# IIT-PAVIS/Acoustic-Image-Generation

Hardware: AMD Instinct MI355X
Metric: train-step images/sec (higher is better)
Workload: dtype f32

## Files before the change

acoustic-image-generation_amd/acimg/_lib.py:

```python
import ctypes as C
import os

_HERE = os.path.dirname(os.path.abspath(__file__))
LIB_PATH = os.environ.get("ACIMG_LIB") or os.path.join(_HERE, "lib", "libacimg.so")

ACT_NONE, ACT_RELU, ACT_SIGMOID = 0, 1, 2


class ConvDesc(C.Structure):

    _fields_ = [(n, C.c_int32) for n in (
        "N", "H", "W", "C", "ldx", "K", "ldy", "OH", "OW", "R", "S", "stride", "pad_t", "pad_l",
        "ldw", "act")]

    def __repr__(self):
        return "ConvDesc(" + ", ".join("%s=%d" % (n, getattr(self, n)) for n, _ in self._fields_) + ")"


class Config(C.Structure):

    _fields_ = [(n, C.c_int32) for n in (
        "splitk_cut", "splitk_target", "splitk_handoff", "wgrad_minpix", "wgrad_halo", "split3_tile_bm",
        "split3_tile_bn", "tail_split", "tail_s", "trunk_persistent", "trunk_bk", "trunk_stagger", "trunk_dma_pos",
        "trunk_ring", "trunk_ring_bm", "trunk_halo")]
# ... 29 lines not shown
    "acimg_conv2d_fwd_tiling": (_I, [_DP, C.POINTER(C.c_int)]),
    "acimg_config_default": (_I, [C.POINTER(Config)]),
    "acimg_configure": (_I, [C.POINTER(Config)]),
    "acimg_conv2d_fwd_workspace": (_SZ, [_DP]),
    "acimg_conv2d_split3_weight_bytes": (_SZ, [_DP]),
    "acimg_conv2d_split3_prepare": (_I, [_DP, _P, _P, _P]),
    "acimg_conv2d_bf16_prepare": (_I, [_DP, _P, _P, _P]),
    "acimg_conv2d_fwd_split3_stats_rows": (_I, [_DP]),
    "acimg_conv2d_fwd_split3_tiling": (_I, [_DP, C.POINTER(C.c_int)]),
    "acimg_conv2d_fwd_split3p_stats_rows": (_I, [_DP]),
    "acimg_conv2d_fwd_split3": (_I, [_DP, _P, _P, _P, _P, _P, _P, _I, _P, _P]),
    "acimg_conv2d_fwd_bf16": (_I, [_DP, _P, _P, _P, _P, _P, _P, _I, _P, _P]),
    "acimg_conv2d_split3_dgrad_weight_bytes": (_SZ, [_DP]),
    "acimg_conv2d_split3_prepare_dgrad": (_I, [_DP, _P, _P, _P]),
    "acimg_conv2d_dgrad_split3": (_I, [_DP, _P, _I, _P, _P, _I, _P, _I, _P, _I, _P]),
    "acimg_conv2d_dgrad_bf16": (_I, [_DP, _P, _I, _P, _P, _I, _P, _I, _P, _I, _P]),
    "acimg_conv2d_split3_prepare_multi": (_I, [_I, _P, _P, _P, _P, _P]),
    "acimg_conv2d_fwd_split3p_workspace": (_SZ, [_DP]),
    "acimg_conv2d_fwd_split3p": (_I, [_DP, _P, _SZ, _P, _P, _P, _P, _SZ, _P]),
    "acimg_conv2d_fwd_split1p": (_I, [_DP, _P, _SZ, _P, _P, _P, _P, _SZ, _P]),
    "acimg_conv2d_fwd_split3p_stats": (_I, [_DP, _P, _SZ, _P, _P, _P, _SZ, _P]),
    "acimg_gram_stats_workspace": (_SZ, [_L, _I]),
    "acimg_gram_stats": (_I, [_P, _SZ, _L, _I, _P, _I, _I, _P, _P, _P, _P, _F, _F, _P, _P, _P, _SZ, _P]),
    "acimg_conv2d_fwd_split3p_tail": (_I, [_DP, _P, _SZ, _P, _P, _P, _P, _SZ, _P, _SZ, _P, _SZ, _P]),
    "acimg_conv2d_fwd_split3p_tail_proj": (_I, [_DP, _P, _SZ, _P, _P, _P, _P, _P, _P, _P, _SZ, _P, _SZ, _P]),
    "acimg_split_plane_bytes": (_SZ, [_L, _I]),
    "acimg_bn_relu_split": (_I, [_P, _P, _P, _I, _P, _SZ, _L, _I, _P]),
    "acimg_bn_add_relu_split": (_I, [_P, _P, _P, _P, _P, _P, _P, _SZ, _P, _SZ, _P, _I, _I, _I, _I, _I, _I, _I, _P]),
    "acimg_bn_relu_maxpool_split": (_I, [_P, _P, _P, _P, _SZ, _I, _I, _I, _I, _I, _I, _I, _I, _P]),
    "acimg_conv2d_dgrad": (_I, [_DP, _P, _I, _P, _P, _I, _P, _I, _P, _I, _P, _SZ, _P, _P]),
    "acimg_conv2d_dgrad_workspace": (_SZ, [_DP]),
    "acimg_conv2d_wgrad": (_I, [_DP, _P, _P, _I, _P, _P, _P, _SZ, _P]),
    "acimg_conv2d_wgrad_workspace": (_SZ, [_DP]),
    "acimg_conv2d_wgrad_split3": (_I, [_DP, _P, _P, _I, _P, _P, _P, _SZ, _P]),
    "acimg_conv2d_wgrad_bf16": (_I, [_DP, _P, _P, _I, _P, _P, _P, _SZ, _P]),
    "acimg_conv2d_affine_input_ok": (_I, [_DP, _I]),
    "acimg_conv2d_wgrad_affine": (_I, [_DP, _I, _P, _P, _P, _I, _P, _I, _P, _P, _P, _SZ, _P]),
    "acimg_deconv_fwd": (_I, [_DP, _P, _P, _P, _P, _P, _SZ, _P, _P]),
    "acimg_deconv_dgrad": (_I, [_DP, _P, _I, _P, _P, _P, _I, _P, _SZ, _P, _P]),
    "acimg_deconv_wgrad": (_I, [_DP, _P, _P, _I, _P, _P, _P, _SZ, _P]),
    "acimg_deconv_workspace": (_SZ, [_DP]),
    "acimg_bn_finalize": (_I, [_P, _I, _I, _I, _D, _P, _P, _P, _P, _F, _F, _I, _P, _P, _P, _P, _P]),
    "acimg_bn_add_relu": (_I, [_P, _P, _P, _P, _P, _P, _P, _I, _I, _I, _I, _I, _I, _I, _P]),
    "acimg_bn_relu_maxpool": (_I, [_P, _P, _P, _P, _I, _I, _I, _I, _I, _I, _I, _I, _P]),
    "acimg_bn_relu": (_I, [_P, _P, _P, _P, _L, _I, _I, _I, _P]),
    "acimg_bn_relu_bwd": (_I, [_P, _P, _P, _P, _P, _P, _P, _P, _P, _L, _I, _P]),
# ... 155 lines not shown
```

acoustic-image-generation_amd/acimg/ops.py:

```python
import ctypes as C
import math

import torch

from . import _lib
from ._lib import ACT_NONE, ACT_RELU, ACT_SIGMOID, ConvDesc


def up4(v):
    return (int(v) + 3) & ~3


class Ptr(object):

    __slots__ = ("t", "off")

    def __init__(self, t, off=0):
        self.t = t
        self.off = int(off)

    def addr(self):
        return self.t.data_ptr() + 4 * self.off


# ... 432 lines not shown
    nbytes = 0 if tail_ws is None else (tail_ws.numel() * tail_ws.element_size() if hasattr(tail_ws, "numel") else 0)
    fn = _L().acimg_conv2d_fwd_split3p if terms == 3 else _L().acimg_conv2d_fwd_split1p
    plan.add("conv2d_fwd_split3p" if terms == 3 else "conv2d_fwd_split1p", fn, C.byref(d), x_planes, int(x_lo_off),
             wsplit, y, stats, tail_ws, int(nbytes), side=side)


def conv2d_fwd_split3p_stats(plan, d, x_planes, x_lo_off, wsplit, stats, tail_ws=None, side=False):
    nbytes = 0 if tail_ws is None else (tail_ws.numel() * tail_ws.element_size() if hasattr(tail_ws, "numel") else 0)
    plan.add("conv2d_fwd_split3p_stats", _L().acimg_conv2d_fwd_split3p_stats, C.byref(d), x_planes, int(x_lo_off), wsplit,
             stats, tail_ws, int(nbytes), side=side)


def gram_stats_workspace(rows, Cn):
    return int(_L().acimg_gram_stats_workspace(int(rows), int(Cn)))


def gram_stats(plan, x_planes, x_lo_off, rows, Cn, w, ldw, K, gamma, beta, moving_mean, moving_var, scale, shift, ws,
               decay=0.997, eps=1e-5, side=False):
    plan.add("gram_stats", _L().acimg_gram_stats, x_planes, int(x_lo_off), int(rows), int(Cn), w, int(ldw), int(K), gamma,
             beta, moving_mean, moving_var, float(decay), float(eps), scale, shift, ws,
             int(ws.numel() * ws.element_size()), side=side)


def conv2d_fwd_split3p_tail(plan, d, x_planes, x_lo_off, wsplit, scale, shift, sc_planes, sc_lo_off, out_planes,
                            out_lo_off, tail_ws=None, side=False):
    nbytes = 0 if tail_ws is None else (tail_ws.numel() * tail_ws.element_size() if hasattr(tail_ws, "numel") else 0)
    plan.add("conv2d_fwd_split3p_tail", _L().acimg_conv2d_fwd_split3p_tail, C.byref(d), x_planes, int(x_lo_off), wsplit,
             scale, shift, sc_planes, int(sc_lo_off), out_planes, int(out_lo_off), tail_ws, int(nbytes), side=side)


def conv2d_fwd_split3p_tail_proj(plan, d, x_planes, x_lo_off, wsplit, scale, shift, sc32, sc_scale, sc_shift, out_planes,
                                 out_lo_off, tail_ws=None, side=False):
    nbytes = 0 if tail_ws is None else (tail_ws.numel() * tail_ws.element_size() if hasattr(tail_ws, "numel") else 0)
    plan.add("conv2d_fwd_split3p_tail_proj", _L().acimg_conv2d_fwd_split3p_tail_proj, C.byref(d), x_planes, int(x_lo_off),
             wsplit, scale, shift, sc32, sc_scale, sc_shift, out_planes, int(out_lo_off), tail_ws, int(nbytes), side=side)


def bn_relu_split(plan, x, scale, shift, relu, out, lo_off, rows, Cn):
    plan.add("bn_relu_split", _L().acimg_bn_relu_split, x, scale, shift, int(relu), out, int(lo_off), int(rows), Cn)


def bn_add_relu_split(plan, a, sa, ta, b32, sb, tb, b_planes, b_lo_off, out_planes, out_lo_off, out32, N, OH, OW,
                      Cn, BH, BW, bstride):
    plan.add("bn_add_relu_split", _L().acimg_bn_add_relu_split, a, sa, ta, b32, sb, tb, b_planes, int(b_lo_off),
             out_planes, int(out_lo_off), out32, N, OH, OW, Cn, BH, BW, bstride)

# ... 364 lines not shown
```

acoustic-image-generation_amd/acimg/vision.py:

```python
from collections import OrderedDict, namedtuple

import numpy as np
import torch

from . import ops
from .model import Model, flat_ptr, load_state_file
from .params import Var, up4

BLOCKS = (("block1", 64, 3, 1), ("block2", 128, 4, 2), ("block3", 256, 6, 2), ("block4", 512, 3, 1))
WEIGHT_DECAY = 5e-4
BN_DECAY = 0.997
BN_EPS = 1e-5
PLANE_SLACK = 2 * 15 * 2048 * 2 + 512

Stage = namedtuple("Stage", "tag a b p1 p2 r1 r2 r3 sc")


class ResNet50Model(Model):

    def __init__(self, input_shape=None, num_classes=None, precision="f16x3", stages=None, stage_cut=8, side_lane=True,
                 two_pass=True, two_pass_max_cin=256, gram=True):
        self.scope = 'resnet_v1_50'
        assert precision in ("f16x3", "f32", "f16")
        self.precision = precision
        self._split = precision in ("f16x3", "f16")
        self._terms = 1 if precision == "f16" else 3
        if stages is None:
            stages = 2 if precision in ("f16x3", "f16") else 1
        assert stages in (1, 2)
        if precision not in ("f16x3", "f16"):
            stages = 1
        self.stages = stages
        self.STAGE_CUT = int(stage_cut)
        self.side_lane = bool(side_lane) and stages == 1
        self.two_pass = bool(two_pass) and precision == "f16x3"
        self.two_pass_max_cin = int(two_pass_max_cin)
        self.gram = bool(gram) and self.two_pass
        self._ctor = dict(input_shape=list(input_shape), num_classes=num_classes, precision=precision, stages=stages,
                          stage_cut=int(stage_cut), side_lane=bool(side_lane), two_pass=bool(two_pass),
                          two_pass_max_cin=int(two_pass_max_cin), gram=bool(gram))
        self.num_classes = num_classes
        self.height = input_shape[0]
        self.width = input_shape[1]
        self.channels = input_shape[2]
        if num_classes is not None:
            raise NotImplementedError("the logits layer is not on the acoustic-image path (num_classes=None)")
        self.session = None
        self.output = None
        self.network = None
        self.frozen_calls = None
        self.stage_calls = None
        self.stage_read_calls = None

    def clone_kwargs(self):
        return dict(self._ctor)

    def _units(self):
        depth_in = 64
        for name, base, n, stride in BLOCKS:
            for u in range(n):
                s = stride if u == n - 1 else 1
                yield ("%s/%s/unit_%d/bottleneck_v1" % (self.scope, name, u + 1), depth_in, base * 4, base, s)
                depth_in = base * 4
# ... 200 lines not shown
                 save=False):
        d = ops.conv_desc(self.N, hw[0], hw[1], cin, cout, kh, kw, stride, padding, ldx=cin, ldy=up4(cout),
                          ldw=up4(cout))
        rows = ops.conv2d_stats_rows(d)
        stats = self._lane_stats("", rows * 2 * up4(cout))
        isc, ish = (in_aff if in_aff is not None else (None, None))
        ops.conv2d_fwd(plan, d, x, self._var(scope + "/weights"), None, out, isc, ish, 1, stats if training else None)
        sc, sh = self._bn_finalize(plan, scope, cout, stats, rows, self.N * d.OH * d.OW, training, save=save)
        return d.OH, d.OW, sc, sh

    def _conv_bn_planes(self, plan, scope, xplanes, hw, cin, kh, kw, cout, stride, padding, out, training, side=False,
                        tag=""):
        d = ops.conv_desc(self.N, hw[0], hw[1], cin, cout, kh, kw, stride, padding, ldx=cin, ldy=up4(cout),
                          ldw=up4(cout))
        rows = ops.conv2d_fwd_split3p_stats_rows(d) if self._terms == 3 else ops.conv2d_fwd_split3_stats_rows(d)
        lane = ("_side" if side else "") + tag
        stats = self._lane_stats(lane, rows * 2 * up4(cout))
        tail_ws = self._lane_ws("tail", lane, ops.conv2d_fwd_split3p_workspace(d))
        ops.conv2d_fwd_split3p(plan, d, xplanes, self._lo_off(self.N * hw[0] * hw[1], cin), self._split_image(scope, d),
                               out, stats if training else None, tail_ws=tail_ws, terms=self._terms, side=side)
        sc, sh = self._bn_finalize(plan, scope, cout, stats, rows, self.N * d.OH * d.OW, training, side=side)
        return d.OH, d.OW, sc, sh

    def _conv3_two_pass(self, plan, scope, xplanes, hw, cin, cout, sc_planes, out_planes, training, tag="", proj=None):
        d = ops.conv_desc(self.N, hw[0], hw[1], cin, cout, 1, 1, 1, "SAME", ldx=cin, ldy=cout, ldw=cout)
        M = self.N * hw[0] * hw[1]
        rows = -(-M // 128)
        stats = self._lane_stats(tag, rows * 2 * cout)
        wsplit = self._split_image(scope, d)
        tail_ws = self._lane_ws("tail", tag, ops.conv2d_fwd_split3p_workspace(d))
        lo = self._lo_off(M, cin)
        lo_out = self._lo_off(M, cout)
        if training and self.gram and ops.gram_stats_workspace(M, cin) > 0:
            sc, sh = self._affine(scope, cout)
            b = scope + "/BatchNorm/"
            ops.gram_stats(plan, xplanes, lo, M, cin, self._var(scope + "/weights"), cout, cout, self._var(b + "gamma"),
                           self._var(b + "beta"), self._var(b + "moving_mean"), self._var(b + "moving_variance"), sc, sh,
                           self._lane_ws("gram", tag, ops.gram_stats_workspace(M, cin)), BN_DECAY, BN_EPS)
        else:
            if training:
                ops.conv2d_fwd_split3p_stats(plan, d, xplanes, lo, wsplit, stats, tail_ws=tail_ws)
            sc, sh = self._bn_finalize(plan, scope, cout, stats, rows, M, training)
        if proj is not None:
            ops.conv2d_fwd_split3p_tail_proj(plan, d, xplanes, lo, wsplit, sc, sh, proj[0], proj[1], proj[2], out_planes,
                                             lo_out, tail_ws=tail_ws)
        else:
            ops.conv2d_fwd_split3p_tail(plan, d, xplanes, lo, wsplit, sc, sh, sc_planes, lo_out, out_planes, lo_out,
                                        tail_ws=tail_ws)

    def _two_pass_ok(self, hw, cin, cout):
        M = self.N * hw[0] * hw[1]
        if not (self.two_pass and self._terms == 3 and cin <= self.two_pass_max_cin and cout % 128 == 0 and
                M * cout * 4 < 2 ** 31):
            return False
        d = ops.conv_desc(self.N, hw[0], hw[1], cin, cout, 1, 1, 1, "SAME", ldx=cin, ldy=cout, ldw=cout)
        return tuple(ops.conv2d_fwd_split3_tiling(d)[:2]) == (128, 128)

    def _record_forward_split(self, plan, training):
        N = self.N
        H, W = self.height, self.width
        plan.add_hook(self._refresh_split_weights)
# ... 20 lines not shown
            def shortcut_conv(side):
                _, _, ssc, tsc = self._conv_bn_planes(plan, scope + "/shortcut", cur, (h, w), din, 1, 1, d, s, "SAME",
                                                      st.sc, training, side=side, tag=st.tag)
                return st.sc, ssc, tsc

            beside = din != d and self.side_lane
            if beside:
                plan.fork()
                forked = shortcut_conv(True)

            def shortcut():
                if din == d:
                    return None
                if beside:
                    plan.join()
                    return forked
                return shortcut_conv(False)

            oh1, ow1, s1, t1 = self._conv_bn_planes(plan, scope + "/conv1", cur, (h, w), din, 1, 1, db, 1, "SAME",
                                                    st.r1, training, tag=st.tag)
            ops.bn_relu_split(plan, st.r1, s1, t1, 1, st.p1, self._lo_off(N * h * w, db), N * h * w, db)
            oh2, ow2, s2, t2 = self._conv_bn_planes(plan, scope + "/conv2", st.p1, (h, w), db, 3, 3, db, s,
                                                    "SAME" if s == 1 else 1, st.r2, training, tag=st.tag)
            ops.bn_relu_split(plan, st.r2, s2, t2, 1, st.p2, self._lo_off(N * oh2 * ow2, db), N * oh2 * ow2, db)
            if s == 1 and not last and self._two_pass_ok((oh2, ow2), db, d):
                self._conv3_two_pass(plan, scope + "/conv3", st.p2, (oh2, ow2), db, d, cur, nxt_out, training, tag=st.tag,
                                     proj=shortcut())
            else:
                _, _, s3, t3 = self._conv_bn_planes(plan, scope + "/conv3", st.p2, (oh2, ow2), db, 1, 1, d, 1, "SAME",
                                                    st.r3, training, tag=st.tag)
                out_planes = None if last else nxt_out
                out_lo = 0 if last else self._lo_off(N * oh2 * ow2, d)
                out32 = self.xfinal if last else None
                proj = shortcut()
                if proj is not None:
                    ops.bn_add_relu_split(plan, st.r3, s3, t3, proj[0], proj[1], proj[2], None, 0, out_planes, out_lo,
                                          out32, N, oh2, ow2, d, oh2, ow2, 1)
                else:
                    ops.bn_add_relu_split(plan, st.r3, s3, t3, None, None, None, cur, self._lo_off(N * h * w, din),
                                          out_planes, out_lo, out32, N, oh2, ow2, d, h, w, s)
            h, w = oh2, ow2
            if i == first2:
                if training:
                    self.stage_read_calls = len(plan.calls)
                cur, nxt = st.a, st.b
            else:
                cur, nxt = nxt, cur
        fh, fw = self.feat_hw
        if training:
            self.frozen_calls = len(plan.calls)
# ... 100 lines not shown
```

acoustic-image-generation_amd/csrc/gram.hip:

```cpp
#include "split_planes.hpp"

namespace acimg {

struct GramParams {
    const char* X;
    unsigned x_bytes;
    unsigned lo_off;
    int rows;
    int C;
    int nb;
    int S;
    int steps;
    float* part;
    float* sxpart;
};

template <int NCC>
__device__ __forceinline__ h16x8 gram_frag(const char* region, int ct, int h, int lane) {
    const int t = lane & 15, q = t >> 2, p = t & 3, g = lane >> 4;
    const int brick = ((2 * h + (g >> 1)) * NCC + (ct >> 1)) * 1024;
    const int kc = 2 * (ct & 1) + (p >> 1);
    const int row0 = 8 * (g & 1) + q, row1 = row0 + 4;
    const int a0 = brick + row0 * 64 + ((kc ^ swz(row0)) << 4) + 8 * (p & 1);
    const int a1 = brick + row1 * 64 + ((kc ^ swz(row1)) << 4) + 8 * (p & 1);
    return tr16_frag<h16x8>(region + a0, region + a1);
}

template <int BC>
__global__ __launch_bounds__(512, 2) void gram_partial_kernel(const GramParams p) {
    constexpr int NCC = BC / 32;
    constexpr int KPB = 4;
    constexpr int REG = KPB * NCC * 1024;
    constexpr int NSD = BC == 128 ? 4 : 3, NSN = 3;
    constexpr int WGN = 4;
    constexpr int TM = BC / 2 / 16, TN = BC / WGN / 16;
    constexpr int PWD = 2 * KPB * NCC / 8;
    constexpr int PWN = 3 * KPB * NCC / 8;
    static_assert(BC == 128 || BC == 64, "block side");

    extern __shared__ __attribute__((aligned(16))) float smem[];
    char* const lds = reinterpret_cast<char*>(smem);
    const int tid = threadIdx.x, lane = tid & 63, wid = tid >> 6;
    const int wm = wid / WGN, wn = wid % WGN;
    const int li = lane & 15, g = lane >> 4;

    const int nb2 = p.nb * p.nb;
    const int xcd = blockIdx.x & 7, slot = blockIdx.x >> 3;
    const int s = xcd + 8 * (slot / nb2), b = slot % nb2;
    if (s >= p.S) return;
    const int bi = b / p.nb, bj = b % p.nb;
    const bool diag = BC == 64 || bi == bj;
// ... 17 lines not shown
    const int STAGE = diag ? 2 * REG : 3 * REG;
    int islot = 0;
    auto issue = [&](int t) {
        char* st = lds + islot * STAGE;
        islot = islot + 1 == NS ? 0 : islot + 1;
#pragma unroll
        for (int j = 0; j < PWN; ++j) {
            if (j >= PWD && diag) break;
            const int p16 = pb0 + KPB * t + pc_pb[j];
            const unsigned goff = (t < p.steps && 16 * p16 + (lane >> 2) < p.rows) ? pc_goff[j] + (unsigned)p16 * cpb * 1024u
                                                                                    : OOB;
            char* dst = st + pc_dst[j];
            __builtin_amdgcn_raw_ptr_buffer_load_lds(rs, (lds_ptr_t)dst, 16, goff, 0, 0, 0);
        }
    };

    f32x4 acc[TM][TN], accs[TN];
#pragma unroll
    for (int j = 0; j < TN; ++j) {
        accs[j] = f32x4{0.f, 0.f, 0.f, 0.f};
#pragma unroll
        for (int i = 0; i < TM; ++i) acc[i][j] = f32x4{0.f, 0.f, 0.f, 0.f};
    }
    const _Float16 one = (_Float16)1.f, half = (_Float16)0.5f;
    const h16x8 ones = {one, one, one, one, one, one, one, one};
    const h16x8 halves = {half, half, half, half, half, half, half, half};
    const bool sums = bi == 0 && wm == 0;

    for (int t = 0; t < NS - 1; ++t) issue(t);
    int cslot = 0;
    for (int t = 0; t < p.steps; ++t) {
        if (diag) wait_vmcnt<(NSD - 2) * PWD>();
        else wait_vmcnt<(NSN - 2) * PWN>();
        __builtin_amdgcn_s_barrier();
        issue(t + NS - 1);
        const char* st = lds + cslot * STAGE;
        cslot = cslot + 1 == NS ? 0 : cslot + 1;
        const char* sta = diag ? st : st + 2 * REG;
#pragma unroll
        for (int h = 0; h < KPB / 2; ++h) {
            h16x8 ah[TM], bh[TN], bl2[TN];
#pragma unroll
            for (int i = 0; i < TM; ++i) ah[i] = gram_frag<NCC>(sta, wm * TM + i, h, lane);
#pragma unroll
            for (int j = 0; j < TN; ++j) {
                bh[j] = gram_frag<NCC>(st, wn * TN + j, h, lane);
                bl2[j] = gram_frag<NCC>(st + REG, wn * TN + j, h, lane) * (_Float16)2.f;
            }
#pragma unroll
            for (int i = 0; i < TM; ++i)
#pragma unroll
                for (int j = 0; j < TN; ++j)
                    acc[i][j] = __builtin_amdgcn_mfma_f32_16x16x32_f16(bl2[j], ah[i], acc[i][j], 0, 0, 0);
#pragma unroll
            for (int i = 0; i < TM; ++i)
#pragma unroll
                for (int j = 0; j < TN; ++j)
                    acc[i][j] = __builtin_amdgcn_mfma_f32_16x16x32_f16(bh[j], ah[i], acc[i][j], 0, 0, 0);
            if (sums) {
#pragma unroll
                for (int j = 0; j < TN; ++j) {
                    accs[j] = __builtin_amdgcn_mfma_f32_16x16x32_f16(bl2[j], halves, accs[j], 0, 0, 0);
                    accs[j] = __builtin_amdgcn_mfma_f32_16x16x32_f16(bh[j], ones, accs[j], 0, 0, 0);
                }
            }
        }
    }
    asm volatile("s_waitcnt vmcnt(0)" ::: "memory");
    float* const out = p.part + ((long)s * nb2 + b) * (BC * BC);
#pragma unroll
    for (int i = 0; i < TM; ++i)
#pragma unroll
        for (int j = 0; j < TN; ++j) {
            const int c1 = (wm * TM + i) * 16 + li, c2 = (wn * TN + j) * 16 + 4 * g;
            *reinterpret_cast<f32x4*>(out + c1 * BC + c2) = acc[i][j];
        }
    if (sums && li == 0) {
#pragma unroll
        for (int j = 0; j < TN; ++j)
            *reinterpret_cast<f32x4*>(p.sxpart + (long)s * p.C + bj * BC + (wn * TN + j) * 16 + 4 * g) = accs[j];
    }
}

__global__ __launch_bounds__(256) void gram_reduce_kernel(const float* part, const float* sxpart, int S, int nb, int BC, int C,
                                                          float* V, float* sx) {
    constexpr int EPB = 8, SG = 32;
    __shared__ double red[SG][EPB][4];
    const int e = threadIdx.x & (EPB - 1), sg = threadIdx.x / EPB;
    const int nmat = C * C / 4 / EPB;
    double a0 = 0.0, a1 = 0.0, a2 = 0.0, a3 = 0.0;
    long dst = -1;
    float scale_back = 0.f;
    if ((int)blockIdx.x < nmat) {
        const int idx = blockIdx.x * EPB + e;
        const int per = BC * BC / 4;
        const int blk = idx / per, w = idx - blk * per;
        const int c1 = w / (BC / 4), c24 = w - c1 * (BC / 4);
        const long stride = (long)nb * nb * BC * BC;
        const float* src = part + (long)blk * BC * BC + (long)c1 * BC + c24 * 4;
        for (int s = sg; s < S; s += SG) {
            const float4 v = *reinterpret_cast<const float4*>(src + s * stride);
            a0 += v.x; a1 += v.y; a2 += v.z; a3 += v.w;
        }
        dst = (long)((blk / nb) * BC + c1) * C + (blk % nb) * BC + c24 * 4;
        scale_back = 1.f / (SPLIT3_ASCALE * SPLIT3_ASCALE);
// ... 95 lines not shown
    size_t off_sx, off_V, off_sxr, bytes;
};
static GramPlan gram_plan(long rows, int C) {
    GramPlan g{};
    g.BC = C % 128 == 0 ? 128 : 64;
    g.nb = C / g.BC;
    g.nblk16 = (int)((rows + 15) / 16);
    int target = g.BC == 128 ? 256 : 512;
    int S = target / (g.nb * g.nb);
    const int max_s = (g.nblk16 + 7) / 8;
    if (S > max_s) S = max_s;
    S = (S + 7) / 8 * 8;
    if (S < 8) S = 8;
    g.S = S;
    g.steps = (g.nblk16 + 4 * S - 1) / (4 * S);
    const size_t part = (size_t)S * g.nb * g.nb * g.BC * g.BC * 4;
    g.off_sx = part;
    g.off_V = g.off_sx + (size_t)S * C * 4;
    g.off_sxr = g.off_V + (size_t)C * C * 4;
    g.bytes = g.off_sxr + (size_t)C * 4;
    return g;
}

}

using namespace acimg;

extern "C" {

size_t acimg_gram_stats_workspace(long rows, int C) {
    if (rows <= 0 || C < 64 || (C != 64 && (C % 128 || C > 512))) return 0;
    return gram_plan(rows, C).bytes;
}

int acimg_gram_stats(const void* x_planes, size_t x_lo_off, long rows, int C, const float* w, int ldw, int K,
                     const float* gamma, const float* beta, float* moving_mean, float* moving_var, float decay, float eps,
                     float* scale, float* shift, void* ws, size_t ws_bytes, void* stream) {
    if (!x_planes || !w || !scale || !shift || !ws || rows <= 0 || K <= 0 || ldw < K)
        return fail(ACIMG_EINVAL, "gram_stats: null argument or bad shape");
    if (C != 64 && (C % 128 || C > 512)) return fail(ACIMG_EINVAL, "gram_stats: C must be 64 or a multiple of 128 up to 512");
    const size_t plane = acimg_split_plane_bytes(rows, C);
    if (!aligned16(x_planes) || (x_lo_off & 15) || x_lo_off < plane || x_lo_off + plane >= (size_t)1 << 31)
        return fail(ACIMG_EINVAL, "gram_stats: unaligned / overlapping / >= 2 GiB split-format input");
    if (!aligned16(ws) || !aligned16(w) || (ldw & 3)) return fail(ACIMG_EINVAL, "gram_stats: unaligned workspace / weights");
    const GramPlan g = gram_plan(rows, C);
    if (ws_bytes < g.bytes) return fail(ACIMG_EINVAL, "gram_stats: workspace too small (%zu < %zu)", ws_bytes, g.bytes);
    char* base = static_cast<char*>(ws);
    GramParams p{};
    p.X = static_cast<const char*>(x_planes);
    p.x_bytes = (unsigned)(x_lo_off + plane);
    p.lo_off = (unsigned)x_lo_off;
    p.rows = (int)rows;
    p.C = C;
    p.nb = g.nb;
    p.S = g.S;
    p.steps = g.steps;
    p.part = reinterpret_cast<float*>(base);
    p.sxpart = reinterpret_cast<float*>(base + g.off_sx);
    float* V = reinterpret_cast<float*>(base + g.off_V);
    float* sxr = reinterpret_cast<float*>(base + g.off_sxr);
    hipStream_t st = (hipStream_t)stream;
    const int grid = g.S * g.nb * g.nb;
    if (g.BC == 128) {
        constexpr int lds = 9 * 4 * 4 * 1024;
        static bool attr = false;
        if (!attr) {
            (void)hipFuncSetAttribute(reinterpret_cast<const void*>(gram_partial_kernel<128>),
                                      hipFuncAttributeMaxDynamicSharedMemorySize, lds);
            attr = true;
        }
        hipLaunchKernelGGL(gram_partial_kernel<128>, dim3(grid), dim3(512), lds, st, p);
    } else {
        constexpr int lds = 6 * 4 * 2 * 1024;
        hipLaunchKernelGGL(gram_partial_kernel<64>, dim3(grid), dim3(512), lds, st, p);
    }
    int rc = check_launch("gram_stats (partials)");
    if (rc) return rc;
    hipLaunchKernelGGL(gram_reduce_kernel, dim3(C * C / 32 + cdiv(C, 32)), dim3(256), 0, st, p.part, p.sxpart, g.S, g.nb, g.BC, C,
                       V, sxr);
    rc = check_launch("gram_stats (reduce)");
    if (rc) return rc;
    const int nw = C >= 256 ? 16 : C / 16;
    const int lds3 = 16 * (C + 4) * 4 + (nw * 64 + nw * 4 * 16) * 8;
#define ACIMG_QUADFIN(CC)                                                                                                  \
    hipLaunchKernelGGL(gram_quadfin_kernel<CC>, dim3(cdiv(K, 16)), dim3(nw * 64), lds3, st, V, sxr, w, ldw, K, (double)rows, \
                       gamma, beta, moving_mean, moving_var, decay, eps, scale, shift)
    if (C == 64) ACIMG_QUADFIN(64);
    else if (C == 128) ACIMG_QUADFIN(128);
    else if (C == 256) ACIMG_QUADFIN(256);
    else if (C == 384) ACIMG_QUADFIN(384);
    else ACIMG_QUADFIN(512);
#undef ACIMG_QUADFIN
    return check_launch("gram_stats (quadratic forms)");
}

}
```

include/acimg.h:

```cpp
#ifndef ACIMG_H_
#define ACIMG_H_

#include <stddef.h>
#include <stdint.h>

#ifdef __cplusplus
extern "C" {
#endif

#define ACIMG_VERSION 207

#define ACIMG_OK 0
#define ACIMG_EINVAL (-1)
#define ACIMG_EWORKSPACE (-2)
#define ACIMG_ELAUNCH (-3)

#define ACIMG_ACT_NONE 0
#define ACIMG_ACT_RELU 1
#define ACIMG_ACT_SIGMOID 2

int acimg_version(void);
int acimg_last_error(char* buf, size_t len);

typedef struct AcimgConvDesc {
// ... 55 lines not shown
int acimg_conv2d_dgrad_bf16(const AcimgConvDesc* d, const float* gy, int ldgy, const void* wsplit_t, float* dx,
                            int lddx, const float* residual, int ldres, const float* mask, int ldmask,
                            void* stream);

size_t acimg_conv2d_fwd_split3p_workspace(const AcimgConvDesc* d);
int acimg_conv2d_fwd_split3p_stats_rows(const AcimgConvDesc* d);
int acimg_conv2d_fwd_split3p(const AcimgConvDesc* d, const void* x_planes, size_t x_lo_off, const void* wsplit,
                             float* y, float* stats, void* ws, size_t ws_bytes, void* stream);
int acimg_conv2d_fwd_split1p(const AcimgConvDesc* d, const void* x_planes, size_t x_lo_off, const void* wsplit,
                             float* y, float* stats, void* ws, size_t ws_bytes, void* stream);
int acimg_conv2d_fwd_split3p_stats(const AcimgConvDesc* d, const void* x_planes, size_t x_lo_off, const void* wsplit,
                                   float* stats, void* ws, size_t ws_bytes, void* stream);
int acimg_conv2d_fwd_split3p_tail(const AcimgConvDesc* d, const void* x_planes, size_t x_lo_off, const void* wsplit,
                                  const float* scale, const float* shift, const void* sc_planes, size_t sc_lo_off,
                                  void* out_planes, size_t out_lo_off, void* ws, size_t ws_bytes, void* stream);
int acimg_conv2d_fwd_split3p_tail_proj(const AcimgConvDesc* d, const void* x_planes, size_t x_lo_off, const void* wsplit,
                                       const float* scale, const float* shift, const float* sc32, const float* sc_scale,
                                       const float* sc_shift, void* out_planes, size_t out_lo_off, void* ws, size_t ws_bytes,
                                       void* stream);
size_t acimg_gram_stats_workspace(long rows, int C);
int acimg_gram_stats(const void* x_planes, size_t x_lo_off, long rows, int C, const float* w, int ldw, int K,
                     const float* gamma, const float* beta, float* moving_mean, float* moving_var, float decay, float eps,
                     float* scale, float* shift, void* ws, size_t ws_bytes, void* stream);
size_t acimg_split_plane_bytes(long rows, int C);
int acimg_bn_relu_split(const float* x, const float* scale, const float* shift, int relu, void* out,
                        size_t lo_off, long rows, int C, void* stream);
int acimg_bn_add_relu_split(const float* a, const float* sa, const float* ta, const float* b32,
                            const float* sb, const float* tb, const void* b_planes, size_t b_lo_off,
                            void* out_planes, size_t out_lo_off, float* out32, int N, int OH, int OW, int C,
                            int BH, int BW, int bstride, void* stream);
int acimg_bn_relu_maxpool_split(const float* x, const float* scale, const float* shift, void* out,
                                size_t lo_off, int N, int H, int W, int C, int OH, int OW, int pad_t, int pad_l,
                                void* stream);

int acimg_conv2d_dgrad(const AcimgConvDesc* d, const float* gy, int ldgy, const float* w,
                       float* dx, int lddx, const float* residual, int ldres, const float* mask,
                       int ldmask, void* ws, size_t ws_bytes, void* tickets, void* stream);
size_t acimg_conv2d_dgrad_workspace(const AcimgConvDesc* d);

int acimg_conv2d_wgrad(const AcimgConvDesc* d, const float* x, const float* gy, int ldgy,
                       float* dw, float* db, void* ws, size_t ws_bytes, void* stream);
size_t acimg_conv2d_wgrad_workspace(const AcimgConvDesc* d);
int acimg_conv2d_wgrad_split3(const AcimgConvDesc* d, const float* x, const float* gy, int ldgy,
                              float* dw, float* db, void* ws, size_t ws_bytes, void* stream);
int acimg_conv2d_wgrad_bf16(const AcimgConvDesc* d, const float* x, const float* gy, int ldgy,
                            float* dw, float* db, void* ws, size_t ws_bytes, void* stream);
// ... 226 lines not shown
```

Before: 5258.

## Fuse BN-ReLU split conversion into gram statistics partial kernel

Adds a fused kernel that reads the raw f32 conv2 output, applies BN affine and ReLU, splits the result into hi/lo f16 planes, writes those planes out, and accumulates the gram partials from LDS in the same pass. The ResNet bottleneck path uses it instead of a separate bn_relu_split followed by gram_stats when the row count is above a per-channel threshold. This removes one full write-then-read of the split planes and one kernel launch. In exchange the new kernel carries more register and LDS pressure and has its own prefetch pipeline, and the shared gram sweep code is refactored into helpers.

Result: no change. 5294, median of 6 (+0.7%).

```diff
diff --git a/acoustic-image-generation_amd/acimg/_lib.py b/acoustic-image-generation_amd/acimg/_lib.py
--- a/acoustic-image-generation_amd/acimg/_lib.py
+++ b/acoustic-image-generation_amd/acimg/_lib.py
@@ -75,6 +75,8 @@
     "acimg_conv2d_fwd_split3p_stats": (_I, [_DP, _P, _SZ, _P, _P, _P, _SZ, _P]),
     "acimg_gram_stats_workspace": (_SZ, [_L, _I]),
     "acimg_gram_stats": (_I, [_P, _SZ, _L, _I, _P, _I, _I, _P, _P, _P, _P, _F, _F, _P, _P, _P, _SZ, _P]),
+    "acimg_bn_relu_split_gram_stats": (_I, [_P, _P, _P, _I, _P, _SZ, _L, _I, _P, _I, _I, _P, _P, _P, _P, _F, _F, _P, _P, _P,
+                                            _SZ, _P]),
     "acimg_conv2d_fwd_split3p_tail": (_I, [_DP, _P, _SZ, _P, _P, _P, _P, _SZ, _P, _SZ, _P, _SZ, _P]),
     "acimg_conv2d_fwd_split3p_tail_proj": (_I, [_DP, _P, _SZ, _P, _P, _P, _P, _P, _P, _P, _SZ, _P, _SZ, _P]),
     "acimg_split_plane_bytes": (_SZ, [_L, _I]),
diff --git a/acoustic-image-generation_amd/acimg/ops.py b/acoustic-image-generation_amd/acimg/ops.py
--- a/acoustic-image-generation_amd/acimg/ops.py
+++ b/acoustic-image-generation_amd/acimg/ops.py
@@ -478,6 +478,13 @@
              int(ws.numel() * ws.element_size()), side=side)
 
 
+def bn_relu_split_gram_stats(plan, x, x_scale, x_shift, relu, out, lo_off, rows, Cn, w, ldw, K, gamma, beta, moving_mean,
+                             moving_var, scale, shift, ws, decay=0.997, eps=1e-5):
+    plan.add("bn_relu_split_gram_stats", _L().acimg_bn_relu_split_gram_stats, x, x_scale, x_shift, int(relu), out,
+             int(lo_off), int(rows), int(Cn), w, int(ldw), int(K), gamma, beta, moving_mean, moving_var, float(decay),
+             float(eps), scale, shift, ws, int(ws.numel() * ws.element_size()))
+
+
 def conv2d_fwd_split3p_tail(plan, d, x_planes, x_lo_off, wsplit, scale, shift, sc_planes, sc_lo_off, out_planes,
                             out_lo_off, tail_ws=None, side=False):
     nbytes = 0 if tail_ws is None else (tail_ws.numel() * tail_ws.element_size() if hasattr(tail_ws, "numel") else 0)
diff --git a/acoustic-image-generation_amd/acimg/vision.py b/acoustic-image-generation_amd/acimg/vision.py
--- a/acoustic-image-generation_amd/acimg/vision.py
+++ b/acoustic-image-generation_amd/acimg/vision.py
@@ -17,9 +17,10 @@
 
 
 class ResNet50Model(Model):
+    GRAM_FUSED_MIN_ROWS = {64: 32 * 56 * 75, 128: 32 * 56 * 75, 256: 32 * 28 * 38}
 
     def __init__(self, input_shape=None, num_classes=None, precision="f16x3", stages=None, stage_cut=8, side_lane=True,
-                 two_pass=True, two_pass_max_cin=256, gram=True):
+                 two_pass=True, two_pass_max_cin=256, gram=True, gram_fused=None):
         self.scope = 'resnet_v1_50'
         assert precision in ("f16x3", "f32", "f16")
         self.precision = precision
@@ -36,9 +37,10 @@
         self.two_pass = bool(two_pass) and precision == "f16x3"
         self.two_pass_max_cin = int(two_pass_max_cin)
         self.gram = bool(gram) and self.two_pass
+        self.gram_fused = None if gram_fused is None else bool(gram_fused)
         self._ctor = dict(input_shape=list(input_shape), num_classes=num_classes, precision=precision, stages=stages,
                           stage_cut=int(stage_cut), side_lane=bool(side_lane), two_pass=bool(two_pass),
-                          two_pass_max_cin=int(two_pass_max_cin), gram=bool(gram))
+                          two_pass_max_cin=int(two_pass_max_cin), gram=bool(gram), gram_fused=self.gram_fused)
         self.num_classes = num_classes
         self.height = input_shape[0]
         self.width = input_shape[1]
@@ -285,7 +287,16 @@
         sc, sh = self._bn_finalize(plan, scope, cout, stats, rows, self.N * d.OH * d.OW, training, side=side)
         return d.OH, d.OW, sc, sh
 
-    def _conv3_two_pass(self, plan, scope, xplanes, hw, cin, cout, sc_planes, out_planes, training, tag="", proj=None):
+    def _gram_route(self, M, cin, training):
+        return bool(training and self.gram and ops.gram_stats_workspace(M, cin) > 0)
+
+    def _gram_fused_ok(self, M, cin):
+        if self.gram_fused is False or cin not in self.GRAM_FUSED_MIN_ROWS:
+            return False
+        return bool(self.gram_fused) or M >= self.GRAM_FUSED_MIN_ROWS[cin]
+
+    def _conv3_two_pass(self, plan, scope, xplanes, hw, cin, cout, sc_planes, out_planes, training, tag="", proj=None,
+                        raw=None):
         d = ops.conv_desc(self.N, hw[0], hw[1], cin, cout, 1, 1, 1, "SAME", ldx=cin, ldy=cout, ldw=cout)
         M = self.N * hw[0] * hw[1]
         rows = -(-M // 128)
@@ -294,12 +305,16 @@
         tail_ws = self._lane_ws("tail", tag, ops.conv2d_fwd_split3p_workspace(d))
         lo = self._lo_off(M, cin)
         lo_out = self._lo_off(M, cout)
-        if training and self.gram and ops.gram_stats_workspace(M, cin) > 0:
+        if self._gram_route(M, cin, training):
             sc, sh = self._affine(scope, cout)
             b = scope + "/BatchNorm/"
-            ops.gram_stats(plan, xplanes, lo, M, cin, self._var(scope + "/weights"), cout, cout, self._var(b + "gamma"),
-                           self._var(b + "beta"), self._var(b + "moving_mean"), self._var(b + "moving_variance"), sc, sh,
-                           self._lane_ws("gram", tag, ops.gram_stats_workspace(M, cin)), BN_DECAY, BN_EPS)
+            stats_args = (self._var(scope + "/weights"), cout, cout, self._var(b + "gamma"), self._var(b + "beta"),
+                          self._var(b + "moving_mean"), self._var(b + "moving_variance"), sc, sh,
+                          self._lane_ws("gram", tag, ops.gram_stats_workspace(M, cin)), BN_DECAY, BN_EPS)
+            if raw is not None:
+                ops.bn_relu_split_gram_stats(plan, raw[0], raw[1], raw[2], 1, xplanes, lo, M, cin, *stats_args)
+            else:
+                ops.gram_stats(plan, xplanes, lo, M, cin, *stats_args)
         else:
             if training:
                 ops.conv2d_fwd_split3p_stats(plan, d, xplanes, lo, wsplit, stats, tail_ws=tail_ws)
@@ -366,10 +381,13 @@
             ops.bn_relu_split(plan, st.r1, s1, t1, 1, st.p1, self._lo_off(N * h * w, db), N * h * w, db)
             oh2, ow2, s2, t2 = self._conv_bn_planes(plan, scope + "/conv2", st.p1, (h, w), db, 3, 3, db, s,
                                                     "SAME" if s == 1 else 1, st.r2, training, tag=st.tag)
-            ops.bn_relu_split(plan, st.r2, s2, t2, 1, st.p2, self._lo_off(N * oh2 * ow2, db), N * oh2 * ow2, db)
-            if s == 1 and not last and self._two_pass_ok((oh2, ow2), db, d):
+            two = s == 1 and not last and self._two_pass_ok((oh2, ow2), db, d)
+            fuse = two and self._gram_route(N * oh2 * ow2, db, training) and self._gram_fused_ok(N * oh2 * ow2, db)
+            if not fuse:
+                ops.bn_relu_split(plan, st.r2, s2, t2, 1, st.p2, self._lo_off(N * oh2 * ow2, db), N * oh2 * ow2, db)
+            if two:
                 self._conv3_two_pass(plan, scope + "/conv3", st.p2, (oh2, ow2), db, d, cur, nxt_out, training, tag=st.tag,
-                                     proj=shortcut())
+                                     proj=shortcut(), raw=(st.r2, s2, t2) if fuse else None)
             else:
                 _, _, s3, t3 = self._conv_bn_planes(plan, scope + "/conv3", st.p2, (oh2, ow2), db, 1, 1, d, 1, "SAME",
                                                     st.r3, training, tag=st.tag)
diff --git a/acoustic-image-generation_amd/csrc/gram.hip b/acoustic-image-generation_amd/csrc/gram.hip
--- a/acoustic-image-generation_amd/csrc/gram.hip
+++ b/acoustic-image-generation_amd/csrc/gram.hip
@@ -27,6 +27,63 @@
 }
 
 template <int BC>
+__device__ __forceinline__ void gram_sweep(const char* st, const char* stl, const char* sta, int wm, int wn, int lane, bool sums,
+                                           f32x4 (&acc)[BC / 32][BC / 64], f32x4 (&accs)[BC / 64]) {
+    constexpr int NCC = BC / 32, KPB = 4, TM = BC / 2 / 16, TN = BC / 4 / 16;
+    const _Float16 one = (_Float16)1.f, half = (_Float16)0.5f;
+    const h16x8 ones = {one, one, one, one, one, one, one, one};
+    const h16x8 halves = {half, half, half, half, half, half, half, half};
+#pragma unroll
+    for (int h = 0; h < KPB / 2; ++h) {
+        h16x8 ah[TM], bh[TN], bl2[TN];
+#pragma unroll
+        for (int i = 0; i < TM; ++i) ah[i] = gram_frag<NCC>(sta, wm * TM + i, h, lane);
+#pragma unroll
+        for (int j = 0; j < TN; ++j) {
+            bh[j] = gram_frag<NCC>(st, wn * TN + j, h, lane);
+            bl2[j] = gram_frag<NCC>(stl, wn * TN + j, h, lane) * (_Float16)2.f;
+        }
+#pragma unroll
+        for (int i = 0; i < TM; ++i)
+#pragma unroll
+            for (int j = 0; j < TN; ++j)
+                acc[i][j] = __builtin_amdgcn_mfma_f32_16x16x32_f16(bl2[j], ah[i], acc[i][j], 0, 0, 0);
+#pragma unroll
+        for (int i = 0; i < TM; ++i)
+#pragma unroll
+            for (int j = 0; j < TN; ++j)
+                acc[i][j] = __builtin_amdgcn_mfma_f32_16x16x32_f16(bh[j], ah[i], acc[i][j], 0, 0, 0);
+        if (sums) {
+#pragma unroll
+            for (int j = 0; j < TN; ++j) {
+                accs[j] = __builtin_amdgcn_mfma_f32_16x16x32_f16(bl2[j], halves, accs[j], 0, 0, 0);
+                accs[j] = __builtin_amdgcn_mfma_f32_16x16x32_f16(bh[j], ones, accs[j], 0, 0, 0);
+            }
+        }
+    }
+}
+
+template <int BC>
+__device__ __forceinline__ void gram_store_partials(const GramParams& p, int s, int b, int bj, int wm, int wn, int li, int g,
+                                                    bool sums, const f32x4 (&acc)[BC / 32][BC / 64],
+                                                    const f32x4 (&accs)[BC / 64]) {
+    constexpr int TM = BC / 2 / 16, TN = BC / 4 / 16;
+    float* const out = p.part + ((long)s * (p.nb * p.nb) + b) * (BC * BC);
+#pragma unroll
+    for (int i = 0; i < TM; ++i)
+#pragma unroll
+        for (int j = 0; j < TN; ++j) {
+            const int c1 = (wm * TM + i) * 16 + li, c2 = (wn * TN + j) * 16 + 4 * g;
+            *reinterpret_cast<f32x4*>(out + c1 * BC + c2) = acc[i][j];
+        }
+    if (sums && li == 0) {
+#pragma unroll
+        for (int j = 0; j < TN; ++j)
+            *reinterpret_cast<f32x4*>(p.sxpart + (long)s * p.C + bj * BC + (wn * TN + j) * 16 + 4 * g) = accs[j];
+    }
+}
+
+template <int BC>
 __global__ __launch_bounds__(512, 2) void gram_partial_kernel(const GramParams p) {
     constexpr int NCC = BC / 32;
     constexpr int KPB = 4;
@@ -90,9 +147,6 @@
 #pragma unroll
         for (int i = 0; i < TM; ++i) acc[i][j] = f32x4{0.f, 0.f, 0.f, 0.f};
     }
-    const _Float16 one = (_Float16)1.f, half = (_Float16)0.5f;
-    const h16x8 ones = {one, one, one, one, one, one, one, one};
-    const h16x8 halves = {half, half, half, half, half, half, half, half};
     const bool sums = bi == 0 && wm == 0;
 
     for (int t = 0; t < NS - 1; ++t) issue(t);
@@ -104,51 +158,17 @@
         issue(t + NS - 1);
         const char* st = lds + cslot * STAGE;
         cslot = cslot + 1 == NS ? 0 : cslot + 1;
-        const char* sta = diag ? st : st + 2 * REG;
-#pragma unroll
-        for (int h = 0; h < KPB / 2; ++h) {
-            h16x8 ah[TM], bh[TN], bl2[TN];
-#pragma unroll
-            for (int i = 0; i < TM; ++i) ah[i] = gram_frag<NCC>(sta, wm * TM + i, h, lane);
-#pragma unroll
-            for (int j = 0; j < TN; ++j) {
-                bh[j] = gram_frag<NCC>(st, wn * TN + j, h, lane);
-                bl2[j] = gram_frag<NCC>(st + REG, wn * TN + j, h, lane) * (_Float16)2.f;
-            }
-#pragma unroll
-            for (int i = 0; i < TM; ++i)
-#pragma unroll
-                for (int j = 0; j < TN; ++j)
-                    acc[i][j] = __builtin_amdgcn_mfma_f32_16x16x32_f16(bl2[j], ah[i], acc[i][j], 0, 0, 0);
-#pragma unroll
-            for (int i = 0; i < TM; ++i)
-#pragma unroll
-                for (int j = 0; j < TN; ++j)
-                    acc[i][j] = __builtin_amdgcn_mfma_f32_16x16x32_f16(bh[j], ah[i], acc[i][j], 0, 0, 0);
-            if (sums) {
-#pragma unroll
-                for (int j = 0; j < TN; ++j) {
-                    accs[j] = __builtin_amdgcn_mfma_f32_16x16x32_f16(bl2[j], halves, accs[j], 0, 0, 0);
-                    accs[j] = __builtin_amdgcn_mfma_f32_16x16x32_f16(bh[j], ones, accs[j], 0, 0, 0);
-                }
-            }
-        }
+        gram_sweep<BC>(st, st + REG, diag ? st : st + 2 * REG, wm, wn, lane, sums, acc, accs);
     }
     asm volatile("s_waitcnt vmcnt(0)" ::: "memory");
-    float* const out = p.part + ((long)s * nb2 + b) * (BC * BC);
-#pragma unroll
-    for (int i = 0; i < TM; ++i)
-#pragma unroll
-        for (int j = 0; j < TN; ++j) {
-            const int c1 = (wm * TM + i) * 16 + li, c2 = (wn * TN + j) * 16 + 4 * g;
-            *reinterpret_cast<f32x4*>(out + c1 * BC + c2) = acc[i][j];
-        }
-    if (sums && li == 0) {
-#pragma unroll
-        for (int j = 0; j < TN; ++j)
-            *reinterpret_cast<f32x4*>(p.sxpart + (long)s * p.C + bj * BC + (wn * TN + j) * 16 + 4 * g) = accs[j];
-    }
-}
+    gram_store_partials<BC>(p, s, b, bj, wm, wn, li, g, sums, acc, accs);
+}
+
+}
+
+#include "gram_fused_kernel.hpp"
+
+namespace acimg {
 
 __global__ __launch_bounds__(256) void gram_reduce_kernel(const float* part, const float* sxpart, int S, int nb, int BC, int C,
                                                           float* V, float* sx) {
@@ -290,34 +310,21 @@
     return g;
 }
 
-}
-
-using namespace acimg;
-
-extern "C" {
-
-size_t acimg_gram_stats_workspace(long rows, int C) {
-    if (rows <= 0 || C < 64 || (C != 64 && (C % 128 || C > 512))) return 0;
-    return gram_plan(rows, C).bytes;
-}
-
-int acimg_gram_stats(const void* x_planes, size_t x_lo_off, long rows, int C, const float* w, int ldw, int K,
-                     const float* gamma, const float* beta, float* moving_mean, float* moving_var, float decay, float eps,
-                     float* scale, float* shift, void* ws, size_t ws_bytes, void* stream) {
-    if (!x_planes || !w || !scale || !shift || !ws || rows <= 0 || K <= 0 || ldw < K)
+static int gram_check(const void* planes, size_t lo_off, long rows, int C, const float* w, int ldw, int K, const float* scale,
+                      const float* shift, void* ws, size_t ws_bytes, GramParams& p) {
+    if (!planes || !w || !scale || !shift || !ws || rows <= 0 || K <= 0 || ldw < K)
         return fail(ACIMG_EINVAL, "gram_stats: null argument or bad shape");
     if (C != 64 && (C % 128 || C > 512)) return fail(ACIMG_EINVAL, "gram_stats: C must be 64 or a multiple of 128 up to 512");
-    const size_t plane = acimg_split_plane_bytes(rows, C);
-    if (!aligned16(x_planes) || (x_lo_off & 15) || x_lo_off < plane || x_lo_off + plane >= (size_t)1 << 31)
+    const size_t plane = split_plane_bytes(rows, C);
+    if (!aligned16(planes) || (lo_off & 15) || lo_off < plane || lo_off + plane >= (size_t)1 << 31)
         return fail(ACIMG_EINVAL, "gram_stats: unaligned / overlapping / >= 2 GiB split-format input");
     if (!aligned16(ws) || !aligned16(w) || (ldw & 3)) return fail(ACIMG_EINVAL, "gram_stats: unaligned workspace / weights");
     const GramPlan g = gram_plan(rows, C);
     if (ws_bytes < g.bytes) return fail(ACIMG_EINVAL, "gram_stats: workspace too small (%zu < %zu)", ws_bytes, g.bytes);
     char* base = static_cast<char*>(ws);
-    GramParams p{};
-    p.X = static_cast<const char*>(x_planes);
-    p.x_bytes = (unsigned)(x_lo_off + plane);
-    p.lo_off = (unsigned)x_lo_off;
+    p.X = static_cast<const char*>(planes);
+    p.x_bytes = (unsigned)(lo_off + plane);
+    p.lo_off = (unsigned)lo_off;
     p.rows = (int)rows;
     p.C = C;
     p.nb = g.nb;
@@ -325,28 +332,17 @@
     p.steps = g.steps;
     p.part = reinterpret_cast<float*>(base);
     p.sxpart = reinterpret_cast<float*>(base + g.off_sx);
+    return 0;
+}
+
+static int gram_finish(const GramPlan& g, const GramParams& p, long rows, int C, const float* w, int ldw, int K,
+                       const float* gamma, const float* beta, float* moving_mean, float* moving_var, float decay, float eps,
+                       float* scale, float* shift, char* base, hipStream_t st) {
     float* V = reinterpret_cast<float*>(base + g.off_V);
     float* sxr = reinterpret_cast<float*>(base + g.off_sxr);
-    hipStream_t st = (hipStream_t)stream;
-    const int grid = g.S * g.nb * g.nb;
-    if (g.BC == 128) {
-        constexpr int lds = 9 * 4 * 4 * 1024;
-        static bool attr = false;
-        if (!attr) {
-            (void)hipFuncSetAttribute(reinterpret_cast<const void*>(gram_partial_kernel<128>),
-                                      hipFuncAttributeMaxDynamicSharedMemorySize, lds);
-            attr = true;
-        }
-        hipLaunchKernelGGL(gram_partial_kernel<128>, dim3(grid), dim3(512), lds, st, p);
-    } else {
-        constexpr int lds = 6 * 4 * 2 * 1024;
-        hipLaunchKernelGGL(gram_partial_kernel<64>, dim3(grid), dim3(512), lds, st, p);
-    }
-    int rc = check_launch("gram_stats (partials)");
-    if (rc) return rc;
     hipLaunchKernelGGL(gram_reduce_kernel, dim3(C * C / 32 + cdiv(C, 32)), dim3(256), 0, st, p.part, p.sxpart, g.S, g.nb, g.BC, C,
                        V, sxr);
-    rc = check_launch("gram_stats (reduce)");
+    const int rc = check_launch("gram_stats (reduce)");
     if (rc) return rc;
     const int nw = C >= 256 ? 16 : C / 16;
     const int lds3 = 16 * (C + 4) * 4 + (nw * 64 + nw * 4 * 16) * 8;
@@ -363,3 +359,85 @@
 }
 
 }
+
+using namespace acimg;
+
+extern "C" {
+
+size_t acimg_gram_stats_workspace(long rows, int C) {
+    if (rows <= 0 || C < 64 || (C != 64 && (C % 128 || C > 512))) return 0;
+    return gram_plan(rows, C).bytes;
+}
+
+int acimg_gram_stats(const void* x_planes, size_t x_lo_off, long rows, int C, const float* w, int ldw, int K,
+                     const float* gamma, const float* beta, float* moving_mean, float* moving_var, float decay, float eps,
+                     float* scale, float* shift, void* ws, size_t ws_bytes, void* stream) {
+    GramParams p{};
+    const int bad = gram_check(x_planes, x_lo_off, rows, C, w, ldw, K, scale, shift, ws, ws_bytes, p);
+    if (bad) return bad;
+    const GramPlan g = gram_plan(rows, C);
+    char* base = static_cast<char*>(ws);
+    hipStream_t st = (hipStream_t)stream;
+    const int grid = g.S * g.nb * g.nb;
+    if (g.BC == 128) {
+        constexpr int lds = 9 * 4 * 4 * 1024;
+        static bool attr = false;
+        if (!attr) {
+            (void)hipFuncSetAttribute(reinterpret_cast<const void*>(gram_partial_kernel<128>),
+                                      hipFuncAttributeMaxDynamicSharedMemorySize, lds);
+            attr = true;
+        }
+        hipLaunchKernelGGL(gram_partial_kernel<128>, dim3(grid), dim3(512), lds, st, p);
+    } else {
+        constexpr int lds = 6 * 4 * 2 * 1024;
+        hipLaunchKernelGGL(gram_partial_kernel<64>, dim3(grid), dim3(512), lds, st, p);
+    }
+    const int rc = check_launch("gram_stats (partials)");
+    if (rc) return rc;
+    return gram_finish(g, p, rows, C, w, ldw, K, gamma, beta, moving_mean, moving_var, decay, eps, scale, shift, base, st);
+}
+
+int acimg_bn_relu_split_gram_stats(const float* x, const float* x_scale, const float* x_shift, int relu, void* out,
+                                   size_t lo_off, long rows, int C, const float* w, int ldw, int K, const float* gamma,
+                                   const float* beta, float* moving_mean, float* moving_var, float decay, float eps,
+                                   float* scale, float* shift, void* ws, size_t ws_bytes, void* stream) {
+    if (!x || !out || (x_scale != nullptr) != (x_shift != nullptr))
+        return fail(ACIMG_EINVAL, "bn_relu_split_gram_stats: null argument");
+    if (!aligned16(x) || !aligned16(x_scale) || !aligned16(x_shift))
+        return fail(ACIMG_EINVAL, "bn_relu_split_gram_stats: unaligned x / scale / shift");
+    GramParams p{};
+    const int rc = gram_check(out, lo_off, rows, C, w, ldw, K, scale, shift, ws, ws_bytes, p);
+    if (rc) return rc;
+    const GramPlan g = gram_plan(rows, C);
+    GramFusedParams f{};
+    f.g = p;
+    f.x = x;
+    f.x_bytes = (unsigned)((size_t)rows * C * 4);
+    f.scale = x_scale;
+    f.shift = x_shift;
+    f.relu = relu;
+    f.out = static_cast<char*>(out);
+    hipStream_t st = (hipStream_t)stream;
+    const int grid = g.S * g.nb * g.nb;
+#define ACIMG_FUSED(BC, NOP, PF)                                                                                          \
+    do {                                                                                                                  \
+        constexpr int lds = 2 * (NOP + 1) * 4 * (BC / 32) * 1024 + NOP * 2 * BC * 4;                                      \
+        static bool attr = false;                                                                                         \
+        if (!attr) {                                                                                                      \
+            (void)hipFuncSetAttribute(reinterpret_cast<const void*>(bn_split_gram_partial_kernel<BC, NOP, PF>),           \
+                                      hipFuncAttributeMaxDynamicSharedMemorySize, lds);                                   \
+            attr = true;                                                                                                  \
+        }                                                                                                                 \
+        hipLaunchKernelGGL((bn_split_gram_partial_kernel<BC, NOP, PF>), dim3(grid), dim3(512), lds, st, f);               \
+    } while (0)
+    if (g.BC == 64) ACIMG_FUSED(64, 1, 2);
+    else if (g.nb == 1) ACIMG_FUSED(128, 1, 2);
+    else ACIMG_FUSED(128, 2, 1);
+#undef ACIMG_FUSED
+    const int rc2 = check_launch("bn_relu_split_gram_stats (split + partials)");
+    if (rc2) return rc2;
+    return gram_finish(g, p, rows, C, w, ldw, K, gamma, beta, moving_mean, moving_var, decay, eps, scale, shift,
+                       static_cast<char*>(ws), st);
+}
+
+}
diff --git a/acoustic-image-generation_amd/csrc/gram_fused_kernel.hpp b/acoustic-image-generation_amd/csrc/gram_fused_kernel.hpp
--- /dev/null
+++ b/acoustic-image-generation_amd/csrc/gram_fused_kernel.hpp
@@ -0,0 +1,155 @@
+#pragma once
+#include <type_traits>
+
+namespace acimg {
+
+struct GramFusedParams {
+    GramParams g;
+    const float* x;
+    unsigned x_bytes;
+    const float* scale;
+    const float* shift;
+    int relu;
+    char* out;
+};
+
+template <int BC, int NOP, int PF>
+__global__ __launch_bounds__(512, 2) void bn_split_gram_partial_kernel(const GramFusedParams p) {
+    constexpr int NCC = BC / 32, KPB = 4, REG = KPB * NCC * 1024;
+    constexpr int STAGE = (NOP + 1) * REG;
+    constexpr int NBW = KPB * NCC / 8;
+    constexpr int WGN = 4;
+    constexpr int TM = BC / 2 / 16, TN = BC / WGN / 16;
+    static_assert(BC == 128 || BC == 64, "block side");
+    static_assert(PF == 1 || PF == 2, "steps in flight");
+
+    extern __shared__ __attribute__((aligned(16))) float smem[];
+    char* const lds = reinterpret_cast<char*>(smem);
+    float* const stash = reinterpret_cast<float*>(lds + 2 * STAGE);
+    const int tid = threadIdx.x, lane = tid & 63, wid = tid >> 6;
+    const int wm = wid / WGN, wn = wid % WGN;
+    const int li = lane & 15, g = lane >> 4;
+
+    const int nb2 = p.g.nb * p.g.nb;
+    const int xcd = blockIdx.x & 7, slot = blockIdx.x >> 3;
+    const int s = xcd + 8 * (slot / nb2), b = slot % nb2;
+    if (s >= p.g.S) return;
+    const int bi = b / p.g.nb, bj = b % p.g.nb;
+    const bool diag = NOP == 1 || bi == bj;
+    const int nop = diag ? 1 : 2;
+    const int pb0 = s * KPB * p.g.steps;
+    const unsigned cpb = (unsigned)p.g.C >> 5;
+    const bool affine = p.scale != nullptr;
+
+    if (affine) {
+        for (int i = tid; i < nop * BC; i += 512) {
+            const int o = i / BC, c = i - o * BC, cg = (o ? bi : bj) * BC + c;
+            stash[o * 2 * BC + c] = p.scale[cg];
+            stash[o * 2 * BC + BC + c] = p.shift[cg];
+        }
+    }
+
+    const __amdgpu_buffer_rsrc_t rs = __builtin_amdgcn_make_buffer_rsrc(const_cast<float*>(p.x), 0, p.x_bytes, 0x00020000);
+    const int row = lane >> 2, kc = lane & 3;
+    const int cc = wid % NCC;
+    const unsigned in_brick = (unsigned)(row * 64 + ((kc ^ swz(row)) << 4));
+    const int cl = cc * 32 + kc * 8;
+
+    f32x4 v[PF][NOP][NBW][2];
+    auto request = [&](int t, auto slot_c) {
+        constexpr int sl = decltype(slot_c)::value;
+#pragma unroll
+        for (int o = 0; o < NOP; ++o) {
+            if (o >= nop) break;
+#pragma unroll
+            for (int j = 0; j < NBW; ++j) {
+                const int pix = 16 * (pb0 + KPB * t + (wid + 8 * j) / NCC) + row;
+                const unsigned off = (t < p.g.steps && pix < p.g.rows)
+                                         ? ((unsigned)pix * (unsigned)p.g.C + (unsigned)((o ? bi : bj) * BC + cl)) * 4u
+                                         : OOB;
+                v[sl][o][j][0] = __builtin_bit_cast(f32x4, __builtin_amdgcn_raw_buffer_load_b128(rs, off, 0, 0));
+                v[sl][o][j][1] = __builtin_bit_cast(f32x4, __builtin_amdgcn_raw_buffer_load_b128(rs, off + 16u, 0, 0));
+            }
+        }
+    };
+    auto convert = [&](int t, auto slot_c) {
+        constexpr int sl = decltype(slot_c)::value;
+        char* const st = lds + (t & 1) * STAGE;
+#pragma unroll
+        for (int o = 0; o < NOP; ++o) {
+            if (o >= nop) break;
+            float4 s0, s1, t0, t1;
+            if (affine) {
+                const float* q = stash + o * 2 * BC + cl;
+                s0 = *reinterpret_cast<const float4*>(q);
+                s1 = *reinterpret_cast<const float4*>(q + 4);
+                t0 = *reinterpret_cast<const float4*>(q + BC);
+                t1 = *reinterpret_cast<const float4*>(q + BC + 4);
+            }
+#pragma unroll
+            for (int j = 0; j < NBW; ++j) {
+                const int pb = (wid + 8 * j) / NCC;
+                const int p16 = pb0 + KPB * t + pb;
+                const bool valid = t < p.g.steps && 16 * p16 + row < p.g.rows;
+                float4 a = __builtin_bit_cast(float4, v[sl][o][j][0]), c = __builtin_bit_cast(float4, v[sl][o][j][1]);
+                if (affine) {
+                    a = affine4(a, s0, t0);
+                    c = affine4(c, s1, t1);
+                }
+                if (p.relu) {
+                    a = relu4(a);
+                    c = relu4(c);
+                }
+                uint2 h0, l0, h1, l1;
+                split4_scaled(scale4(a, SPLIT3_ASCALE), h0, l0);
+                split4_scaled(scale4(c, SPLIT3_ASCALE), h1, l1);
+                uint4 hi = make_uint4(h0.x, h0.y, h1.x, h1.y), lo = make_uint4(l0.x, l0.y, l1.x, l1.y);
+                if (!valid) hi = lo = make_uint4(0u, 0u, 0u, 0u);
+                const unsigned at = (unsigned)((pb * NCC + cc) * 1024) + in_brick;
+                if (o == 0) {
+                    *reinterpret_cast<uint4*>(st + at) = hi;
+                    *reinterpret_cast<uint4*>(st + REG + at) = lo;
+                    if (diag && valid) {
+                        const size_t go = ((size_t)p16 * cpb + (unsigned)(bj * NCC + cc)) * 1024u + in_brick;
+                        *reinterpret_cast<uint4*>(p.out + go) = hi;
+                        *reinterpret_cast<uint4*>(p.out + p.g.lo_off + go) = lo;
+                    }
+                } else {
+                    *reinterpret_cast<uint4*>(st + 2 * REG + at) = hi;
+                }
+            }
+        }
+    };
+    using S0 = std::integral_constant<int, 0>;
+    using S1 = std::integral_constant<int, PF - 1>;
+
+    f32x4 acc[TM][TN], accs[TN];
+#pragma unroll
+    for (int j = 0; j < TN; ++j) {
+        accs[j] = f32x4{0.f, 0.f, 0.f, 0.f};
+#pragma unroll
+        for (int i = 0; i < TM; ++i) acc[i][j] = f32x4{0.f, 0.f, 0.f, 0.f};
+    }
+    const bool sums = bi == 0 && wm == 0;
+
+    request(0, S0{});
+    if (PF == 2) request(1, S1{});
+    __syncthreads();
+    convert(0, S0{});
+    auto step = [&](int t, auto cur_c) {
+        __syncthreads();
+        request(t + PF, cur_c);
+        const char* st = lds + (t & 1) * STAGE;
+        gram_sweep<BC>(st, st + REG, diag ? st : st + 2 * REG, wm, wn, lane, sums, acc, accs);
+    };
+    for (int t = 0; t + 1 < p.g.steps; t += 2) {
+        step(t, S0{});
+        convert(t + 1, S1{});
+        step(t + 1, S1{});
+        convert(t + 2, S0{});
+    }
+    if (p.g.steps & 1) step(p.g.steps - 1, S0{});
+    gram_store_partials<BC>(p.g, s, b, bj, wm, wn, li, g, sums, acc, accs);
+}
+
+}
diff --git a/include/acimg.h b/include/acimg.h
--- a/include/acimg.h
+++ b/include/acimg.h
@@ -101,6 +101,10 @@
 int acimg_gram_stats(const void* x_planes, size_t x_lo_off, long rows, int C, const float* w, int ldw, int K,
                      const float* gamma, const float* beta, float* moving_mean, float* moving_var, float decay, float eps,
                      float* scale, float* shift, void* ws, size_t ws_bytes, void* stream);
+int acimg_bn_relu_split_gram_stats(const float* x, const float* x_scale, const float* x_shift, int relu, void* out,
+                                   size_t lo_off, long rows, int C, const float* w, int ldw, int K, const float* gamma,
+                                   const float* beta, float* moving_mean, float* moving_var, float decay, float eps,
+                                   float* scale, float* shift, void* ws, size_t ws_bytes, void* stream);
 size_t acimg_split_plane_bytes(long rows, int C);
 int acimg_bn_relu_split(const float* x, const float* scale, const float* shift, int relu, void* out,
                         size_t lo_off, long rows, int C, void* stream);
```
